# troubling/hummingbird

Measured on AMD Instinct MI355X. Metric: GiB/s device-resident EC encode+reconstruct, 4+2 @ 1 MiB; % HBM roofline, higher is better.
Workload: dtype u8; 1 GPU; 4+2 Encode + Reconstruct{0,1} of 4096 x 1 MiB objects per GPU, device-resident (BASELINE configs[1]+[2]); k=4, m=2, object_bytes=1048576, objects_per_gpu=4096, global_objects=4096, parallelism=object-partition x1

## Files before the change

hummingbird_amd/_native.py:

```python
from __future__ import annotations

import ctypes as C
import os
from pathlib import Path

_PKG = Path(__file__).resolve().parent
LIB_PATH = Path(os.environ.get("HBEC_LIB", _PKG / "libhbec.so"))

HBEC_OK = 0
ERR_INV_SHARD_NUM = -1
ERR_MAX_SHARD_NUM = -2
ERR_TOO_FEW_SHARDS = -3
ERR_SHARD_NO_DATA = -4
ERR_SHARD_SIZE = -5
ERR_SINGULAR = -6
ERR_INVALID_ARG = -7
ERR_DEVICE = -8
ERR_NOMEM = -9
ERR_UNEXPECTED_EOF = -10
ERR_IO = -11
ERR_SCHEME = -12

LOC_BAD = 0x80000000
LOC_SKIPPED = 0x40000000
# ... 73 lines not shown
    ("hbec_plan_stripes", C.c_int, [_P, C.POINTER(Stripe), C.c_uint64, C.POINTER(_P)]),
    ("hbec_plan_objects", C.c_int, [_P, C.POINTER(Object), C.c_uint64, C.POINTER(_P)]),
    ("hbec_plan_free", None, [_P]),
    ("hbec_plan_info", C.c_int,
     [_P, C.POINTER(C.c_uint64), C.POINTER(C.c_int), C.POINTER(C.c_uint64), C.POINTER(C.c_uint64)]),
    ("hbec_encode_plan", C.c_int, [_P, _P, _P]),
    ("hbec_reconstruct_plan", C.c_int, [_P, _P, _U8P, C.c_int, _P]),
    ("hbec_reconstruct_plan_mixed", C.c_int, [_P, _P, _U8P, C.c_uint32, C.POINTER(C.c_uint32), C.c_int, _P]),
    ("hbec_mixed_plan_stats", C.c_int, [C.POINTER(C.c_uint64), C.POINTER(C.c_uint64)]),
    ("hbec_mixed_plan_tile_bytes", C.c_int, []),
    ("hbec_set_mixed_plan_chunk_tiles", C.c_int, [C.c_uint64]),
    ("hbec_verify_plan", C.c_int, [_P, _P, _P, _P]),
    ("hbec_verify_plan_stats", C.c_int, [C.POINTER(C.c_uint64), C.POINTER(C.c_uint64)]),
    ("hbec_verify_plan_tile_bytes", C.c_int, [C.c_int]),
    ("hbec_verify_plan_mixed", C.c_int, [_P, _P, _U8P, C.c_uint32, C.POINTER(C.c_uint32), _P, _P]),
    ("hbec_check_rows", C.c_int,
     [_P, _U8P, C.POINTER(C.c_int), C.POINTER(C.c_int), C.POINTER(C.c_int), _U8P]),
    ("hbec_verify_mixed_plan_stats", C.c_int, [C.POINTER(C.c_uint64), C.POINTER(C.c_uint64)]),
    ("hbec_verify_mixed_plan_tile_bytes", C.c_int, []),
    ("hbec_set_verify_mixed_plan_chunk_tiles", C.c_int, [C.c_uint64]),
    ("hbec_locate_plan_mixed", C.c_int, [_P, _P, _U8P, C.c_uint32, C.POINTER(C.c_uint32), _P, _P, _P]),
    ("hbec_locate_decode", C.c_int, [C.c_int, C.c_int, _U8P, C.c_uint32]),
    ("hbec_locate_plan_stats", C.c_int, [C.POINTER(C.c_uint64), C.POINTER(C.c_uint64)]),
    ("hbec_locate_plan_tile_bytes", C.c_int, []),
    ("hbec_set_locate_plan_chunk_tiles", C.c_int, [C.c_uint64]),
    ("hbec_repair_plan_mixed", C.c_int, [_P, _P, _U8P, C.c_uint32, C.POINTER(C.c_uint32), C.c_int, _P, _P]),
    ("hbec_repair_plan_stats", C.c_int, [C.POINTER(C.c_uint64), C.POINTER(C.c_uint64)]),
    ("hbec_repair_plan_tile_bytes", C.c_int, []),
    ("hbec_set_repair_plan_chunk_tiles", C.c_int, [C.c_uint64]),
    ("hbec_heal_plan_mixed", C.c_int, [_P, _P, _U8P, C.c_uint32, C.POINTER(C.c_uint32), _P, _P, _P]),
    ("hbec_heal_plan_stats", C.c_int, [C.POINTER(C.c_uint64), C.POINTER(C.c_uint64)]),
    ("hbec_heal_plan_tile_bytes", C.c_int, []),
    ("hbec_set_heal_plan_chunk_tiles", C.c_int, [C.c_uint64]),
    ("hbec_verify_host", C.c_int, [_P, C.POINTER(Stripe), C.c_uint64, _U8P]),
    ("hbec_encode_host", C.c_int, [_P, C.POINTER(Stripe), C.c_uint64]),
    ("hbec_host_alloc", C.c_int, [C.c_size_t, C.POINTER(_P)]),
    ("hbec_host_free", None, [_P]),
    ("hbec_host_device_addr", C.c_int, [_P, C.c_uint64, C.POINTER(C.c_uint64)]),
    ("hbec_reconstruct_host", C.c_int, [_P, C.POINTER(Stripe), C.c_uint64, _U8P, C.c_int]),
    ("hbec_encode_host_md5", C.c_int, [_P, C.POINTER(Stripe), C.c_uint64, _U8P]),
    ("hbec_device_count", C.c_int, [C.POINTER(C.c_int)]),
    ("hbec_set_device", C.c_int, [C.c_int]),
    ("hbec_encode_host_devices", C.c_int, [_P, C.POINTER(Stripe), C.c_uint64, C.POINTER(C.c_int), C.c_int]),
    ("hbec_reconstruct_host_devices", C.c_int,
     [_P, C.POINTER(Stripe), C.c_uint64, _U8P, C.c_int, C.POINTER(C.c_int), C.c_int]),
    ("hbec_batcher_new", C.c_int, [_P, C.c_uint64, C.c_uint32, C.POINTER(_P)]),
    ("hbec_batcher_free", None, [_P]),
    ("hbec_batcher_encode", C.c_int, [_P, C.POINTER(Stripe)]),
    ("hbec_batcher_encode_md5", C.c_int, [_P, C.POINTER(Stripe), _U8P]),
    ("hbec_batcher_reconstruct", C.c_int, [_P, C.POINTER(Stripe), _U8P, C.c_int]),
    ("hbec_batcher_stats", C.c_int, [_P, C.POINTER(C.c_uint64), C.POINTER(C.c_uint64)]),
    ("hbec_set_force_stream", C.c_int, [C.c_int]),
    ("hbec_set_odd_chunk_tiles", C.c_int, [C.c_uint64]),
    ("hbec_kernel_info", C.c_int,
     [C.c_int, C.c_int, C.c_uint64, C.POINTER(C.c_int), C.POINTER(C.c_int), C.POINTER(C.c_int)]),
    ("hbec_odd_path_stats", C.c_int, [C.POINTER(C.c_uint64), C.POINTER(C.c_uint64), C.POINTER(C.c_uint64)]),
    ("hbec_verify_route_stats", C.c_int, [C.POINTER(VerifyRoutes)]),
    ("hbec_apply_route_stats", C.c_int, [C.POINTER(ApplyRoutes)]),
    ("hbec_odd_edge_stats", C.c_int, [C.POINTER(C.c_uint64), C.POINTER(C.c_uint64)]),
    ("hbec_odd_record_cache", C.c_int, [C.c_int, C.POINTER(C.c_uint64), C.POINTER(C.c_uint64)]),
    ("hbec_ec_shard_length", C.c_int64, [C.c_int64, C.c_int64]),
    ("hbec_ec_split", C.c_int, [C.c_int, C.c_int, READ_FN, _P, C.c_int, C.c_int64, WRITE_FN, C.POINTER(_P)]),
    ("hbec_ec_reconstruct", C.c_int,
     [C.c_int, C.c_int, READ_FN, C.POINTER(_P), C.c_int, C.c_int64, WRITE_FN, C.POINTER(_P),
      C.POINTER(C.c_int), C.c_int]),
    ("hbec_ec_glue", C.c_int,
     [C.c_int, C.c_int, READ_FN, C.POINTER(_P), C.c_int, C.c_int64, WRITE_FN, C.POINTER(_P), C.c_int]),
    ("hbec_ec_glue_range", C.c_int,
     [C.c_int, C.c_int, READ_FN, C.POINTER(_P), C.c_int, C.c_int64, C.c_int64, C.c_int64, WRITE_FN, C.POINTER(_P),
      C.c_int]),
    ("hbec_ec_copy_range", C.c_int,
     [C.c_int, C.c_int, READ_FN, C.POINTER(_P), C.c_int, C.c_int64, C.c_int64, C.c_int64, WRITE_FN, C.POINTER(_P),
      C.c_int]),
    ("hbec_parse_ec_scheme", C.c_int,
     [C.c_char_p, C.c_char_p, C.c_size_t, C.POINTER(C.c_int64), C.POINTER(C.c_int64), C.POINTER(C.c_int64)]),
    ("hbec_range_chunk_align", None,
     [C.c_int64, C.c_int64, C.c_int64, C.c_int, C.POINTER(C.c_int64), C.POINTER(C.c_int64)]),
]
SYMBOLS = [s[0] for s in _SIG]

_lib = None


class NativeLibraryError(RuntimeError):
    pass


def lib():
    global _lib
    if _lib is None:
        if not LIB_PATH.exists():
            raise NativeLibraryError(
                f"{LIB_PATH} not found: build it with `python -m hummingbird_amd.build` "
                "(there is no CPU fallback)")
        try:
            h = C.CDLL(str(LIB_PATH))
        except OSError as e:
            raise NativeLibraryError(f"cannot load {LIB_PATH}: {e}") from e
        for name, res, args in _SIG:
            if "HBEC_LIB" in os.environ and not hasattr(h, name):
                continue
            fn = getattr(h, name)
            fn.restype = res
            fn.argtypes = args
        _lib = h
    return _lib
# ... 9 lines not shown
```

hummingbird_amd/batch.py:

```python
from __future__ import annotations

import ctypes as C

from . import _native as N
from .reedsolomon import Encoder, check

HBEC_SEED = 0x48424543


def _stream_ptr(stream):
    import torch

    if stream is None:
        stream = torch.cuda.current_stream()
    return C.c_void_p(stream.cuda_stream)


def shard_views(t, n_shards: int, shard_len: int):
    if t.dim() != 2 or t.stride(1) != 1:
        raise ValueError("expected a 2-D row-contiguous tensor")
    if t.shape[1] < n_shards * shard_len:
        raise ValueError("tensor rows shorter than n_shards * shard_len")
    base = t.data_ptr()
    row = t.stride(0) * t.element_size()
# ... 336 lines not shown
    check(N.lib().hbec_mixed_plan_stats(C.byref(a), C.byref(b)))
    return {"kernel_launches": a.value, "per_stripe_calls": b.value}


def mixed_plan_tile_bytes() -> int:
    return int(N.lib().hbec_mixed_plan_tile_bytes())


def set_mixed_plan_chunk_tiles(tiles: int) -> None:
    check(N.lib().hbec_set_mixed_plan_chunk_tiles(int(tiles)))


def verify_mixed_plan_stats():
    a, b = C.c_uint64(), C.c_uint64()
    check(N.lib().hbec_verify_mixed_plan_stats(C.byref(a), C.byref(b)))
    return {"kernel_launches": a.value, "per_stripe_calls": b.value}


def verify_mixed_plan_tile_bytes() -> int:
    return int(N.lib().hbec_verify_mixed_plan_tile_bytes())


def set_verify_mixed_plan_chunk_tiles(tiles: int) -> None:
    check(N.lib().hbec_set_verify_mixed_plan_chunk_tiles(int(tiles)))


KERNEL_KINDS = {0: "unrolled", 1: "pipelined", 2: "streaming", 3: "packed", 4: "records"}


def kernel_info(k: int, r: int, shard_len: int):
    tb, kind, bpc = C.c_int(), C.c_int(), C.c_int()
    check(N.lib().hbec_kernel_info(k, r, int(shard_len), C.byref(tb), C.byref(kind), C.byref(bpc)))
    return {"tile_bytes": tb.value, "kind": KERNEL_KINDS[kind.value], "blocks_per_cu": bpc.value}


def odd_path_stats():
    b, r, s = C.c_uint64(), C.c_uint64(), C.c_uint64()
    check(N.lib().hbec_odd_path_stats(C.byref(b), C.byref(r), C.byref(s)))
    e, f = C.c_uint64(), C.c_uint64()
    check(N.lib().hbec_odd_edge_stats(C.byref(e), C.byref(f)))
    return {"bitplane": b.value, "records": r.value, "strided": s.value, "edges": e.value, "fused": f.value}


def odd_record_cache(clear: bool = False):
    e, h = C.c_uint64(), C.c_uint64()
    check(N.lib().hbec_odd_record_cache(1 if clear else 0, C.byref(e), C.byref(h)))
    return e.value, h.value


def set_odd_chunk_tiles(tiles: int) -> None:
    N.lib().hbec_set_odd_chunk_tiles(int(tiles))


def set_force_stream(on: bool) -> None:
    N.lib().hbec_set_force_stream(1 if on else 0)
```

hummingbird_amd/csrc/hbec.cpp:

```cpp
#include <hip/hip_runtime.h>

#include <algorithm>
#include <atomic>
#include <condition_variable>
#include <cstdio>
#include <cstdlib>
#include <cstring>
#include <deque>
#include <map>
#include <memory>
#include <mutex>
#include <string>
#include <tuple>
#include <vector>

#include "../../include/hbec.h"
#include "gf256.h"
#include "internal.h"
#include "kernels.h"
#include "mixed.h"
#include "vmixed.h"

namespace hbec {

static thread_local std::string t_last_error;

int fail(int code, const std::string& msg) {
    t_last_error = msg;
    return code;
}

int hip_fail(hipError_t e, const char* what) {
    (void)hipGetLastError();
    std::string m = std::string(what) + ": " + hipGetErrorString(e);
    return fail(e == hipErrorOutOfMemory ? HBEC_ERR_NOMEM : HBEC_ERR_DEVICE, m);
}

long long hbec::env_knob(const char* name, long long dflt) {
    const char* e = std::getenv(name);
    return e && *e ? std::atoll(e) : dflt;
}

static std::atomic<int> g_force_stream{0};
static const int g_unaligned_bpc = (int)tune_knob("HBEC_UNALIGNED_BPC", 0);
static const int g_blocks_per_cu_override = (int)tune_knob("HBEC_BLOCKS_PER_CU", 0);
static const int g_grid_cap_env = (int)tune_knob("HBEC_GRID_CAP", 0);
thread_local int t_grid_cap = 0;
void set_thread_grid_cap(int blocks) { t_grid_cap = blocks; }
static int apply_grid_cap(int grid) {
    int cap = g_grid_cap_env;
    if (t_grid_cap > 0) cap = cap > 0 ? std::min(t_grid_cap, cap) : t_grid_cap;
    return cap > 0 ? std::min(grid, cap) : grid;
}
static const uint64_t g_chunk_tiles = [] {
    const long long v = tune_knob("HBEC_CHUNK_TILES", 0);
    return (uint64_t)(v > 0 ? v : (1ll << 20));
}();
static std::atomic<uint64_t> g_odd_chunk_override{0};
static uint64_t odd_chunk_tiles() {
    const uint64_t v = g_odd_chunk_override.load(std::memory_order_relaxed);
    return v ? v : g_chunk_tiles;
}
static const uint64_t g_vec_chunk_tiles = [] {
    const long long v = tune_knob("HBEC_VEC_CHUNK_TILES", tune_knob("HBEC_CHUNK_TILES", 0));
    return (uint64_t)(v > 0 ? v : HBEC_VEC_CHUNK_TILES);
}();

enum class OccKind { Unrolled, Pipelined, ForcedStream, Packed, Unaligned, VerifyPipe, VerifyPacked };

struct DeviceInfo {
    int cus = 0;
    std::map<std::tuple<OccKind, int, int>, int> blocks_per_cu;
};

static std::mutex g_dev_mu;
static std::map<int, DeviceInfo> g_devs;

static int current_device(int* dev) {
    hipError_t e = hipGetDevice(dev);
    if (e != hipSuccess) return hip_fail(e, "hipGetDevice");
    return HBEC_OK;
}

static int device_info(int dev, DeviceInfo** out) {
    DeviceInfo& d = g_devs[dev];
    if (d.cus == 0) {
        hipDeviceProp_t p;
        hipError_t e = hipGetDeviceProperties(&p, dev);
        if (e != hipSuccess) return hip_fail(e, "hipGetDeviceProperties");
        d.cus = p.multiProcessorCount;
    }
    *out = &d;
    return HBEC_OK;
}

int device_cus(int dev, int* cus) {
    std::lock_guard<std::mutex> g(g_dev_mu);
    DeviceInfo* d = nullptr;
    int rc = device_info(dev, &d);
    if (rc) return rc;
    *cus = d->cus;
    return HBEC_OK;
}

static int device_blocks(int dev, OccKind kind, int k, int r, int* cus, int* per_cu) {
    std::lock_guard<std::mutex> g(g_dev_mu);
    DeviceInfo* d = nullptr;
    int rc = device_info(dev, &d);
    if (rc) return rc;
    if (kind == OccKind::Unaligned) k = 0;
    auto it = d->blocks_per_cu.find({kind, k, r});
    if (it == d->blocks_per_cu.end()) {
        int b = 0;
        hipError_t e = hipErrorInvalidValue;
        switch (kind) {
            case OccKind::Unrolled: e = vec_occupancy(k, r, 0, 0, &b); break;
            case OccKind::Pipelined: e = vec_occupancy(k, r, 1, 0, &b); break;
            case OccKind::ForcedStream: e = vec_occupancy(k, r, 0, 1, &b); break;
            case OccKind::Packed: e = packed_occupancy(k, r, &b); break;
// ... 239 lines not shown
                uint64_t n_obj, uint64_t shard_len, hipStream_t stream) {
    if (rows <= 0 || n_obj == 0 || shard_len == 0) return HBEC_OK;
    if (cols <= 0 || !coeffs || !in || !out) return fail(HBEC_ERR_INVALID_ARG, "apply: bad arguments");
    bool vec = vec_len(shard_len);
    for (int c = 0; c < cols && vec; ++c) vec = aligned16(in[c].base) && vec_len(in[c].obj_stride);
    for (int r = 0; r < rows && vec; ++r) vec = aligned16(out[r].base) && vec_len(out[r].obj_stride);
    bool line = vec && shard_len % 128 == 0;
    for (int c = 0; c < cols && line; ++c) line = line_aligned(in[c].base, in[c].obj_stride);
    for (int r = 0; r < rows && line; ++r) line = line_aligned(out[r].base, out[r].obj_stride);
    const bool to_rec = vec && rec_route(cols, rows, shard_len, line, true) &&
                        (rec_route(cols, rows, shard_len, line, false) || bitplane_rows(cols, rows, coeffs, cols, 0, false));
    for (int c = 0; c < cols; ++c)
        if (!in[c].base) return fail(HBEC_ERR_INVALID_ARG, "apply: null input view");
    for (int r = 0; r < rows; ++r)
        if (!out[r].base) return fail(HBEC_ERR_INVALID_ARG, "apply: null output view");
    int dev = 0;
    int rc = current_device(&dev);
    if (rc) return rc;
    const int force_stream = g_force_stream.load();
    if (!vec && cols > kMaxK && cols <= 256 && pos32_shard(shard_len)) {
        count_apply(kArWide);
        return apply_wide(rows, cols, coeffs, in, out, n_obj, shard_len, stream);
    }

    for (int r0 = 0; r0 < rows; r0 += kMaxR) {
        const int R = std::min(kMaxR, rows - r0);
        for (int c0 = 0; c0 < cols; c0 += kMaxK) {
            const int K = std::min(kMaxK, cols - c0);
            PassArgs a = make_pass(in, out, coeffs, cols, r0, R, c0, K, shard_len);
            a.accumulate = c0 > 0 ? 1u : 0u;
            int cus = 0, per_cu = 0;
            if (vec && is_packed_shape(K, R, shard_len, c0 > 0, force_stream)) {
                count_apply(kArPacked);
                rc = device_blocks(dev, OccKind::Packed, K, R, &cus, &per_cu);
                if (rc) return rc;
                if (g_blocks_per_cu_override > 0) per_cu = g_blocks_per_cu_override;
                const uint64_t spo = shard_len / 16;
                const uint64_t te = (uint64_t)packed_tile_elems(K);
                const uint64_t max_obj = packed_objs_per_launch(spo, te, g_chunk_tiles);
                rc = for_object_chunks(a, K, R, n_obj, max_obj, [&](PassArgs& b, uint64_t) {
                    set_packed_tiles(b, spo, te);
                    const int grid = grid_blocks(b.n_tiles, kPipeBlockThreads / 64, (uint64_t)cus * per_cu);
                    return launched(launch_packed(K, R, b, apply_grid_cap(grid), stream), "launch gf_apply_packed");
                });
            } else if (vec && !to_rec) {
                count_apply(kArVec);
                const int pipe = is_pipe_shape(K, R, shard_len, force_stream) && c0 == 0;
                rc = device_blocks(dev, vec_kind(pipe, force_stream), K, R, &cus, &per_cu);
                if (rc) return rc;
                if (g_blocks_per_cu_override > 0) per_cu = g_blocks_per_cu_override;
                const uint64_t tile = (uint64_t)vec_tile_bytes(K, R, shard_len, c0 > 0, force_stream);
                const uint64_t tpo = (shard_len + tile - 1) / tile;
                const uint64_t wpb = (uint64_t)vec_block_threads(K, R, shard_len, c0 > 0, force_stream) / 64;
                const uint64_t max_obj = objs_per_launch(g_vec_chunk_tiles, tpo);
                rc = for_object_chunks(a, K, R, n_obj, max_obj, [&](PassArgs& b, uint64_t) {
                    set_tiles(b, tpo);
                    const int grid = grid_blocks(b.n_tiles, wpb, (uint64_t)cus * per_cu);
                    return launched(launch_vec(K, R, b, apply_grid_cap(grid), stream, force_stream), "launch gf_apply_vec");
                });
            } else if (odd_enabled() && cols <= kOddMaxK && pos32_shard(shard_len)) {
                count_apply(kArOdd);
                rc = odd_launches(a, K, R, 0, c0 > 0, n_obj, shard_len, nullptr, dev, stream);
            } else {
                count_apply(kArUnaligned);
                rc = device_blocks(dev, OccKind::Unaligned, K, R, &cus, &per_cu);
                if (rc) return rc;
                if (g_unaligned_bpc > 0) per_cu = std::min(per_cu, g_unaligned_bpc);
                const uint64_t tpo = unaligned_tiles_per_obj(shard_len);
                const uint64_t max_obj = objs_per_launch(g_chunk_tiles, tpo);
                rc = for_object_chunks(a, K, R, n_obj, max_obj, [&](PassArgs& b, uint64_t) {
                    set_tiles(b, tpo);
                    const int grid = grid_blocks(b.n_tiles, kBlockThreads / 64, (uint64_t)cus * per_cu);
                    return launched(launch_unaligned(K, R, b, apply_grid_cap(grid), stream), "launch gf_apply_unaligned");
                });
            }
            if (rc) return rc;
        }
    }
    return HBEC_OK;
}

struct Staging {
    int dev = 0;
    hipStream_t stream = nullptr;
    uint8_t* dbuf = nullptr;
    size_t dcap = 0;
    uint8_t* hbuf = nullptr;
    uint64_t hbuf_dev = 0;
    size_t hcap = 0;
    std::vector<hipEvent_t> ev;
};

static const bool g_percall_mapped = tune_knob("HBEC_PERCALL_DMA", 0) == 0;

static const int g_percall_pieces = (int)std::max(1LL, std::min(16LL, tune_knob("HBEC_PERCALL_PIECES", 2)));

class PercallGate {
  public:
    explicit PercallGate(int limit) : limit_(limit) {}
    void enter() {
        if (limit_ <= 0) return;
        std::unique_lock<std::mutex> lk(mu_);
        if (running_ < limit_ && waiters_.empty()) {
            ++running_;
            return;
        }
        Waiter w;
        waiters_.push_back(&w);
        w.cv.wait(lk, [&] { return w.granted; });
    }
// ... 995 lines not shown

static void databuf_shards(const hbec_codec* c, uint8_t* databuf, size_t s, std::vector<uint8_t*>& p) {
    p.resize((size_t)(c->k + c->m));
    for (size_t i = 0; i < p.size(); ++i) p[i] = databuf + i * s;
}

int hbec_encode_databuf(hbec_codec* c, uint8_t* databuf, size_t shard_len) {
    return hbec::guarded("hbec_encode_databuf", [&]() -> int {
        if (!c || !databuf) return fail(HBEC_ERR_INVALID_ARG, "null argument");
        if (shard_len == 0) return fail(HBEC_ERR_SHARD_NO_DATA, "no shard data");
        if (coalesce_enabled()) return coalesced_call(c, 0, databuf, shard_len, nullptr, c->k + c->m, 0, kDirect);
        return direct_encode(c, databuf, shard_len);
    });
}

int hbec_reconstruct_databuf(hbec_codec* c, uint8_t* databuf, size_t shard_len, const uint8_t* present,
                             int data_only) {
    return hbec::guarded("hbec_reconstruct_databuf", [&]() -> int {
        if (!c || !databuf || !present) return fail(HBEC_ERR_INVALID_ARG, "null argument");
        std::vector<uint8_t*> p;
        databuf_shards(c, databuf, shard_len, p);
        std::vector<size_t> lens(p.size());
        for (size_t i = 0; i < p.size(); ++i) lens[i] = present[i] ? shard_len : 0;
        return hbec_reconstruct(c, p.data(), lens.data(), (int)p.size(), data_only);
    });
}

int hbec_verify_databuf(hbec_codec* c, const uint8_t* databuf, size_t shard_len, int* ok) {
    return hbec::guarded("hbec_verify_databuf", [&]() -> int {
        if (!c || !databuf || !ok) return fail(HBEC_ERR_INVALID_ARG, "null argument");
        *ok = 0;
        if (shard_len == 0) return fail(HBEC_ERR_SHARD_NO_DATA, "no shard data");
        std::vector<uint8_t*> p;
        databuf_shards(c, const_cast<uint8_t*>(databuf), shard_len, p);
        std::vector<size_t> lens(p.size(), shard_len);
        return hbec_verify(c, p.data(), lens.data(), (int)p.size(), ok);
    });
}

int hbec_coalesce_stats(uint64_t* groups, uint64_t* calls) {
    return hbec::guarded("hbec_coalesce_stats", [&]() -> int {
        coalesce_stats(groups, calls);
        return HBEC_OK;
    });
}

int hbec_set_odd_chunk_tiles(uint64_t tiles) {
    return hbec::guarded("hbec_set_odd_chunk_tiles", [&]() -> int {
        g_odd_chunk_override.store(tiles, std::memory_order_relaxed);
        return HBEC_OK;
    });
}

int hbec_set_force_stream(int on) {
    return hbec::guarded("hbec_set_force_stream", [&]() -> int {
        g_force_stream.store(on ? 1 : 0);
        return HBEC_OK;
    });
}

int hbec_kernel_info(int k, int r, uint64_t shard_len, int* tile_bytes, int* kind, int* blocks_per_cu) {
    return hbec::guarded("hbec_kernel_info", [&]() -> int {
        if (k < 1 || k > kMaxK || r < 1 || r > kMaxR) return fail(HBEC_ERR_INVALID_ARG, "shape out of range");
        const int fs = g_force_stream.load();
        const bool packed = r <= 3 && is_packed_shape(k, r, shard_len, 0, fs);
        const bool rec = !packed && shard_len % 16 == 0 && rec_route(k, r, shard_len, shard_len % 128 == 0, false);
        const int pipe = packed ? 2 : is_pipe_shape(k, r, shard_len, fs);
        if (tile_bytes)
            *tile_bytes = packed ? packed_tile_elems(k) * 16
                                 : (rec ? (int)odd_rec_tile_span(k, 0, -1) : vec_tile_bytes(k, r, shard_len, 0, fs));
        if (kind) *kind = packed ? 3 : (rec ? 4 : (is_streaming_shape(k, r, fs) ? 2 : (pipe ? 1 : 0)));
        if (blocks_per_cu) {
            int dev = 0, cus = 0;
            int rc = current_device(&dev);
            if (rc) return rc;
            rc = device_blocks(dev, packed ? OccKind::Packed : vec_kind(pipe, fs), k, r, &cus, blocks_per_cu);
            if (rc) return rc;
            if (rec) *blocks_per_cu = odd_blocks_per_cu(0, k, r, false, true);
            if (g_blocks_per_cu_override > 0) *blocks_per_cu = g_blocks_per_cu_override;
        }
        return HBEC_OK;
    });
}

}

extern "C" int hbec_odd_record_cache(int clear, uint64_t* entries, uint64_t* hits) {
    return hbec::guarded("hbec_odd_record_cache", [&]() -> int {
        ObjRecCache& C = objrec_cache();
        std::lock_guard<std::mutex> lk(C.mu);
        if (clear) {
            hipError_t e = hipDeviceSynchronize();
            if (e != hipSuccess) return hip_fail(e, "hipDeviceSynchronize (record cache)");
            for (auto& x : C.entries) {
                if (x.ev) (void)hipEventDestroy(x.ev);
                if (x.d) (void)hipFree(x.d);
            }
            C.entries.clear();
            C.seen.clear();
            C.bytes = 0;
            C.hits = 0;
        }
        if (entries) *entries = C.entries.size();
        if (hits) *hits = C.hits;
        return HBEC_OK;
    });
// ... 2 lines not shown
```

hummingbird_amd/csrc/kernels.h:

```cpp
#pragma once
#include <hip/hip_runtime.h>
#include <stdint.h>

#include "tuning.h"

namespace hbec {

long long env_knob(const char* name, long long dflt);
inline long long tune_knob(const char* name, long long dflt) {
#if HBEC_TUNE
    return env_knob(name, dflt);
#else
    (void)name;
    return dflt;
#endif
}

constexpr int kMaxK = 16;
constexpr uint32_t kOddListWords = 4;
constexpr int kMaxR = 4;
constexpr int kBlockThreads = 256;
constexpr int kPipeBlockThreads = HBEC_PIPE_BLOCK;
constexpr int kPipeBlocksPerCu = HBEC_PIPE_BLOCKS_PER_CU;

constexpr int kVecWavesPerSimd = HBEC_WAVES_PER_SIMD;

struct PassArgs {
    const uint8_t* in[kMaxK];
    uint64_t in_stride[kMaxK];
    uint8_t* out[kMaxR];
    uint64_t out_stride[kMaxR];
    uint32_t tab[kMaxR][kMaxK][5];
    uint64_t n_obj;
    uint64_t shard_len;
    uint32_t tiles_per_obj;
    uint32_t n_tiles;
    uint32_t accumulate;
    uint32_t n_elems;
    uint32_t elems_per_obj;
    uint32_t fuse;
    const uint32_t* list;
};

int is_packed_shape(int k, int r, uint64_t shard_len, int accumulate, int force_stream);
int packed_tile_elems(int k);
hipError_t launch_packed(int k, int r, const PassArgs& a, int grid, hipStream_t stream);
hipError_t packed_occupancy(int k, int r, int* blocks_per_cu);

int vec_tile_bytes(int k, int r, uint64_t shard_len, int accumulate, int force_stream);
int is_streaming_shape(int k, int r, int force_stream);
int is_pipe_shape(int k, int r, uint64_t shard_len, int force_stream);
int vec_block_threads(int k, int r, uint64_t shard_len, int accumulate, int force_stream);
__host__ __device__ constexpr int pipe_u(int k) { return k <= 4 ? (4 / k) : (k <= 8 ? HBEC_PIPE_U_BIG : 1); }

__host__ __device__ constexpr int stripes_u(int k) { return k <= 4 ? pipe_u(k) : 1; }
__host__ __device__ constexpr int verify_u(int k) { return k <= 4 ? 4 : 1; }

hipError_t launch_vec(int k, int r, const PassArgs& a, int grid, hipStream_t stream, int force_stream);
uint32_t unaligned_tiles_per_obj(uint64_t shard_len);
hipError_t launch_unaligned(int k, int r, const PassArgs& a, int grid, hipStream_t stream);
hipError_t unaligned_occupancy(int r, int* blocks_per_cu);
struct URec {
    uint64_t a;
    uint64_t b;
    uint64_t shard_len;
    uint64_t p0;
};
struct UPlanArgs {
    const URec* recs;
    uint32_t n_recs;
    uint32_t accumulate;
    uint32_t in_idx[kMaxK];
    uint32_t out_idx[kMaxR];
    uint32_t in_sel, out_sel;
    uint32_t tab[kMaxR][kMaxK][5];
    uint32_t mirror;
    uint32_t carry;
};
uint32_t unaligned_tile_bytes();
hipError_t launch_verify_unaligned(int k, int r, const PassArgs& a, uint32_t* flags, int grid, hipStream_t stream);
hipError_t launch_unaligned_plan(int k, int r, const UPlanArgs& a, int grid, hipStream_t stream);
constexpr int kOddMaxK = 12;
constexpr uint64_t kPos32MaxShard = (1ull << 31) - (1ull << 16);
__host__ __device__ constexpr bool pos32_shard(uint64_t shard_len) { return shard_len <= kPos32MaxShard; }
bool odd_enabled();
int odd_blocks_per_cu(int mode, int k, int r, bool mirror = false, bool records = false, int xs = -1);
bool odd_supported(int k, int r);
uint64_t urec_tile();
uint64_t urec_tile_for(int k, bool mirror);
uint64_t urec_span(uint64_t shard_len);
uint32_t odd_tile_bytes(int k);
uint32_t odd_plan_tile_bytes();
uint32_t odd_tiles_per_obj(int k, int mode, uint64_t shard_len, bool records, int xs = -1);
uint64_t odd_frame_tiles(uint64_t shard_len, uint64_t tile);
int odd_bp_schedule(int k, int r, int mode, const uint32_t (*tab)[kMaxK][5], bool plan);
uint32_t odd_rec_tile_span(int k, int mode, int xs);
uint32_t odd_waves_per_block(int xs);
uint64_t odd_min_main();
bool odd_uses_records(int k, int r);
uint32_t odd_rec_words(int k, int r, int mode);
hipError_t launch_odd_objrec(int k, int r, int mode, const PassArgs& a, uint32_t* recs, hipStream_t stream);
hipError_t launch_odd_planrec(int k, int r, int mode, const UPlanArgs& p, const URec* orecs, uint32_t n,
                              uint32_t* recs, hipStream_t stream);
hipError_t launch_odd(int k, int r, int mode, const PassArgs& a, uint32_t* flags, const uint32_t* recs, int grid,
                      hipStream_t stream, int xs = -1);
bool odd_edge_fuse(int k, int r, int mode, bool records, int xs, bool list, uint64_t max_s);
// ... 80 lines not shown
```

hummingbird_amd/csrc/kernels.hip:

```cpp
#include <hip/hip_runtime.h>
#include <stdint.h>

#include <cstdlib>
#include <cstring>

#include "gf_device.h"
#include "kernels.h"

namespace hbec {

template <int K, int R, int U>
__device__ __forceinline__ void process_tile(const PassArgs& a, const Tables<K, R>& tb, uint64_t obj,
                                             uint64_t off0, bool full, bool accumulate) {
    u32x4 x[U][K];
    const uint64_t last = a.shard_len - 16u;
#pragma unroll
    for (int u = 0; u < U; ++u) {
        uint64_t off = off0 + (uint64_t)u * 1024u;
        if (!full) off = off < last ? off : last;
#pragma unroll
        for (int j = 0; j < K; ++j) x[u][j] = ld16(a.in[j] + obj * a.in_stride[j] + off);
    }
    u32x4 old[U][R];
    if (accumulate) {
// ... 139 lines not shown
#pragma unroll
    for (int r = 0; r < R; ++r) b.out[r] = reinterpret_cast<uint64_t>(a.out[r]) + obj * a.out_stride[r] + off;
    const uint64_t left = a.shard_len - off;
    b.valid = (uint32_t)(left < TILE ? left : TILE);
    b.live = b.valid;
}

template <int K, int R, int U>
__device__ __forceinline__ void pipe2_load(u32x4 (&x)[U][K], const PipeTile<K, R>& b, uint32_t lane) {
    const uint64_t last = (uint64_t)b.valid - 16u;
#pragma unroll
    for (int q = 0; q < U * K; ++q) {
        const int u = HBEC_PIPE_IMAJ ? q % U : q / K, j = HBEC_PIPE_IMAJ ? q / U : q % K;
        uint64_t off = (uint64_t)lane * 16u + (uint64_t)u * 1024u;
        off = off < last ? off : last;
        x[u][j] = HBEC_PIPE_TEMP ? ld16_addr_t(b.in[j] + off) : ld16_addr(b.in[j] + off);
    }
}

template <int K, int R, int U, bool FULL>
__device__ __forceinline__ void pipe2_store_(const u32x4 (&x)[U][K], const PassArgs& a, const Tables<K, R>& tb,
                                             const PipeTile<K, R>& b, uint32_t lane) {
#pragma unroll
    for (int u = 0; u < U; ++u) {
        const uint64_t off = (uint64_t)lane * 16u + (uint64_t)u * 1024u;
        u32x4 acc[R];
#pragma unroll
        for (int r = 0; r < R; ++r) acc[r] = u32x4{0, 0, 0, 0};
        gf_dot<K, R>(acc, x[u], a.tab, tb);
        if (FULL || off < b.live) {
#pragma unroll
            for (int r = 0; r < R; ++r) st16_addr(b.out[r] + off, acc[r]);
        }
    }
}

template <int K, int R, int U>
__device__ __forceinline__ void pipe_tile_at(PipeTile<K, R>& b, const PassArgs& a, uint32_t t, uint32_t n,
                                             uint32_t tpo) {
    pipe_tile_coords<K, R, U>(b, a, t < n ? t : n - 1u, tpo);
    if (t >= n) b.live = 0;
}

template <int K, int R, int U>
__device__ __forceinline__ void pipe2_finish(const u32x4 (&x)[U][K], const PassArgs& a, const Tables<K, R>& tb,
                                             const PipeTile<K, R>& cur, uint32_t lane) {
    if (cur.live >= (uint32_t)U * 1024u)
        pipe2_store_<K, R, U, true>(x, a, tb, cur, lane);
    else
        pipe2_store_<K, R, U, false>(x, a, tb, cur, lane);
}


template <int K, int R>
__global__ __launch_bounds__(kPipeBlockThreads, 1) void gf_apply_vec_pipe2(PassArgs a) {
    constexpr int U = pipe_u(K);
    constexpr uint32_t WPB = kPipeBlockThreads / 64;
    const uint32_t lane = threadIdx.x & 63u;
    const uint32_t nw = gridDim.x * WPB;
    const uint32_t wave0 = __builtin_amdgcn_readfirstlane(xcd_block() * WPB);
    const uint32_t dw = __builtin_amdgcn_readfirstlane(threadIdx.x >> 6);
    const uint32_t wave = wave0 + dw;
    const uint32_t tpo = a.tiles_per_obj;
    const uint32_t n = a.n_tiles;
    if (wave0 >= n) return;
    const Tables<K, R> tb = load_tables<K, R>(a.tab);
    PipeTile<K, R> cur, nxt;
    pipe_tile_at<K, R, U>(cur, a, wave, n, tpo);
    u32x4 x[U][K];
    pipe2_load<K, R, U>(x, cur, lane);
    pipe_tile_at<K, R, U>(nxt, a, wave + nw, n, tpo);
    for (uint32_t b0 = wave0 + nw; b0 < n; b0 += nw) {
        u32x4 y[U][K];
        pipe2_load<K, R, U>(y, nxt, lane);
        if (K <= 4) __builtin_amdgcn_s_sleep(HBEC_PIPE2_SLEEP);
        __builtin_amdgcn_s_barrier();
        PipeTile<K, R> after;
        pipe_tile_at<K, R, U>(after, a, b0 + dw + nw, n, tpo);
        pipe2_finish<K, R, U>(x, a, tb, cur, lane);
#pragma unroll
        for (int u = 0; u < U; ++u)
#pragma unroll
            for (int j = 0; j < K; ++j) x[u][j] = y[u][j];
        cur = nxt;
        nxt = after;
    }
    pipe2_finish<K, R, U>(x, a, tb, cur, lane);
}

template <int K, int U>
__device__ __forceinline__ void packed_load(u32x4 (&x)[U][K], const PassArgs& a, const PackedCoord<U>& c) {
#pragma unroll
    for (int u = 0; u < U; ++u)
#pragma unroll
        for (int j = 0; j < K; ++j) x[u][j] = ld16(a.in[j] + (uint64_t)c.obj[u] * a.in_stride[j] + c.off[u]);
}

template <int K, int R, int U, bool FULL>
__device__ __forceinline__ void packed_store_(const u32x4 (&x)[U][K], const PassArgs& a, const Tables<K, R>& tb,
                                              const PackedCoord<U>& c, uint32_t t, uint32_t lane, uint32_t live) {
#pragma unroll
    for (int u = 0; u < U; ++u) {
        u32x4 acc[R];
#pragma unroll
        for (int r = 0; r < R; ++r) acc[r] = u32x4{0, 0, 0, 0};
        gf_dot<K, R>(acc, x[u], a.tab, tb);
        if (FULL || (t * (uint32_t)U + (uint32_t)u) * 64u + lane < live) {
#pragma unroll
            for (int r = 0; r < R; ++r) st16(a.out[r] + (uint64_t)c.obj[u] * a.out_stride[r] + c.off[u], acc[r]);
        }
    }
}

template <int K, int R, int U>
__device__ __forceinline__ void packed_finish(const u32x4 (&x)[U][K], const PassArgs& a, const Tables<K, R>& tb,
                                              const PackedCoord<U>& c, uint32_t t, uint32_t n, uint32_t lane) {
    const uint32_t live = t < n ? a.n_elems : 0u;
    if (t < n && (t + 1u) * (uint32_t)U * 64u <= a.n_elems)
        packed_store_<K, R, U, true>(x, a, tb, c, t, lane, live);
    else
        packed_store_<K, R, U, false>(x, a, tb, c, t, lane, live);
}


__host__ __device__ constexpr int packed_u(int k) {
    return k > 4 ? HBEC_PACKED_U_BIG : pipe_u(k);
}

template <int K, int R>
__global__ __launch_bounds__(kPipeBlockThreads, 1) void gf_apply_packed(PassArgs a) {
    constexpr int U = packed_u(K);
// ... 572 lines not shown
```

hummingbird_amd/csrc/tuning.h:

```cpp
#pragma once

#ifndef HBEC_TUNE
#define HBEC_TUNE 0
#endif

#ifndef HBEC_PIPE_BLOCK
#define HBEC_PIPE_BLOCK 256
#endif
#ifndef HBEC_PIPE_BLOCKS_PER_CU
#define HBEC_PIPE_BLOCKS_PER_CU 1
#endif
#ifndef HBEC_PIPE_U_BIG
#define HBEC_PIPE_U_BIG 3
#endif
#ifndef HBEC_PIPE_SLEEP
#define HBEC_PIPE_SLEEP 6
#endif
#ifndef HBEC_PIPE2_SLEEP
#define HBEC_PIPE2_SLEEP 8
#endif
#ifndef HBEC_PIPE_IMAJ
#define HBEC_PIPE_IMAJ 0
#endif
#ifndef HBEC_PIPE_TEMP
#define HBEC_PIPE_TEMP 0
#endif
#ifndef HBEC_VEC_CHUNK_TILES
#define HBEC_VEC_CHUNK_TILES 262144
#endif
#ifndef HBEC_PIPE_V2_MAXK
#define HBEC_PIPE_V2_MAXK 4
#endif

#ifndef HBEC_WAVES_PER_SIMD
#define HBEC_WAVES_PER_SIMD 4
#endif
#ifndef HBEC_TILE_SMALL
#define HBEC_TILE_SMALL 4
#endif
#ifndef HBEC_TILE_MID
#define HBEC_TILE_MID 1
#endif
#ifndef HBEC_TILE_BIG
#define HBEC_TILE_BIG 1
#endif

#ifndef HBEC_ALLVGPR_MIN
#define HBEC_ALLVGPR_MIN 16
#endif

#ifndef HBEC_PACKED_U_BIG
#define HBEC_PACKED_U_BIG 1
#endif
#ifndef HBEC_PACKED_MAX_BIG
#define HBEC_PACKED_MAX_BIG 32784
#endif
#ifndef HBEC_PACKED_BLOCKS_SMALL
#define HBEC_PACKED_BLOCKS_SMALL 2
#endif
#ifndef HBEC_PACKED_BLOCKS_BIG
#define HBEC_PACKED_BLOCKS_BIG 1
#endif
#ifndef HBEC_VERIFY_PACKED_U_SMALL
#define HBEC_VERIFY_PACKED_U_SMALL 2
#endif
#ifndef HBEC_VERIFY_PACKED_U_BIG
#define HBEC_VERIFY_PACKED_U_BIG 1
#endif
#ifndef HBEC_VERIFY_PACKED_BLOCKS_SMALL
#define HBEC_VERIFY_PACKED_BLOCKS_SMALL 2
#endif
#ifndef HBEC_VERIFY_PACKED_BLOCKS_BIG
// ... 89 lines not shown
```

include/hbec.h:

```cpp
#ifndef HBEC_H
#define HBEC_H

#include <stddef.h>
#include <stdint.h>

#ifdef __cplusplus
extern "C" {
#endif


#define HBEC_VERSION 2

enum {
    HBEC_OK = 0,
    HBEC_ERR_INV_SHARD_NUM = -1,
    HBEC_ERR_MAX_SHARD_NUM = -2,
    HBEC_ERR_TOO_FEW_SHARDS = -3,
    HBEC_ERR_SHARD_NO_DATA = -4,
    HBEC_ERR_SHARD_SIZE = -5,
    HBEC_ERR_SINGULAR = -6,
    HBEC_ERR_INVALID_ARG = -7,
    HBEC_ERR_DEVICE = -8,
    HBEC_ERR_NOMEM = -9,
    HBEC_ERR_UNEXPECTED_EOF = -10,
// ... 111 lines not shown
#define HBEC_LOC_BAD 0x80000000u
#define HBEC_LOC_SKIPPED 0x40000000u
#define HBEC_LOC_NOTHING 0x20000000u
int hbec_locate_plan_mixed(hbec_codec* codec, const hbec_plan* plan, const uint8_t* patterns, uint32_t n_patterns,
                           const uint32_t* pattern_of, const uint32_t* d_flags ,
                           uint32_t* d_where, void* hip_stream);
#define HBEC_LOC_CLEAN (-1)
#define HBEC_LOC_AMBIGUOUS (-2)
#define HBEC_LOC_MULTIPLE (-3)
#define HBEC_LOC_UNCHECKED (-4)
int hbec_locate_decode(int k, int m, const uint8_t* present, uint32_t where);
int hbec_locate_plan_stats(uint64_t* kernel_launches, uint64_t* skipped_entries);
int hbec_locate_plan_tile_bytes(void);
int hbec_set_locate_plan_chunk_tiles(uint64_t tiles);
int hbec_repair_plan_mixed(hbec_codec* codec, const hbec_plan* plan, const uint8_t* patterns, uint32_t n_patterns,
                           const uint32_t* pattern_of, int data_only, uint32_t* d_flags, void* hip_stream);
int hbec_repair_plan_stats(uint64_t* kernel_launches, uint64_t* per_stripe_calls);
int hbec_repair_plan_tile_bytes(void);
int hbec_set_repair_plan_chunk_tiles(uint64_t tiles);
#define HBEC_HEAL_DONE 4u
#define HBEC_HEAL_UNNAMED 8u
int hbec_heal_plan_mixed(hbec_codec* codec, const hbec_plan* plan, const uint8_t* patterns, uint32_t n_patterns,
                         const uint32_t* pattern_of, const uint32_t* d_where, uint32_t* d_flags, void* hip_stream);
int hbec_heal_plan_stats(uint64_t* kernel_launches, uint64_t* skipped_entries);
int hbec_heal_plan_tile_bytes(void);
int hbec_set_heal_plan_chunk_tiles(uint64_t tiles);

int hbec_encode_host(hbec_codec* codec, const hbec_stripe* stripes, uint64_t n_stripes);
int hbec_host_alloc(size_t bytes, void** out);
void hbec_host_free(void* p);
int hbec_host_device_addr(const void* p, uint64_t len, uint64_t* dev);
int hbec_reconstruct_host(hbec_codec* codec, const hbec_stripe* stripes, uint64_t n_stripes, const uint8_t* present,
                          int data_only);
int hbec_verify_host(hbec_codec* codec, const hbec_stripe* stripes, uint64_t n_stripes, uint8_t* flags);
int hbec_device_count(int* n);
int hbec_set_device(int device);
int hbec_encode_host_devices(hbec_codec* codec, const hbec_stripe* stripes, uint64_t n_stripes, const int* devices,
                             int n_devices);
int hbec_reconstruct_host_devices(hbec_codec* codec, const hbec_stripe* stripes, uint64_t n_stripes,
                                  const uint8_t* present, int data_only, const int* devices, int n_devices);
int hbec_encode_host_md5(hbec_codec* codec, const hbec_stripe* stripes, uint64_t n_stripes, uint8_t* digests);
int hbec_host_md5_stats(uint64_t* zero_copy_calls, uint64_t* ring_calls);

typedef struct hbec_batcher hbec_batcher;
int hbec_batcher_new(hbec_codec* codec, uint64_t max_batch_bytes, uint32_t max_wait_us, hbec_batcher** out);
void hbec_batcher_free(hbec_batcher* batcher);
int hbec_batcher_encode(hbec_batcher* batcher, const hbec_stripe* stripe);
int hbec_batcher_encode_md5(hbec_batcher* batcher, const hbec_stripe* stripe, uint8_t* digests);
int hbec_batcher_reconstruct(hbec_batcher* batcher, const hbec_stripe* stripe, const uint8_t* present, int data_only);
int hbec_batcher_stats(hbec_batcher* batcher, uint64_t* batches, uint64_t* stripes);

int hbec_set_force_stream(int on);
int hbec_set_odd_chunk_tiles(uint64_t tiles);
int hbec_kernel_info(int k, int r, uint64_t shard_len, int* tile_bytes, int* kind, int* blocks_per_cu);
int hbec_odd_path_stats(uint64_t* bitplane, uint64_t* records, uint64_t* strided);
typedef struct hbec_verify_routes {
    uint64_t packed, pipe, records, odd, wide, unaligned, scratch;
} hbec_verify_routes;
int hbec_verify_route_stats(hbec_verify_routes* out);
typedef struct hbec_apply_routes {
    uint64_t packed, vec, odd, unaligned, wide;
} hbec_apply_routes;
int hbec_apply_route_stats(hbec_apply_routes* out);

int hbec_odd_edge_stats(uint64_t* edge_launches, uint64_t* fused_launches);

int hbec_odd_record_cache(int clear, uint64_t* entries, uint64_t* hits);

typedef int64_t (*hbec_read_fn)(void* ctx, uint8_t* buf, size_t n);
typedef int (*hbec_write_fn)(void* ctx, const uint8_t* buf, size_t n);

int64_t hbec_ec_shard_length(int64_t length, int64_t data_shards);

int hbec_ec_split(int data_shards, int parity_shards, hbec_read_fn read, void* fp, int chunk_size,
                  int64_t content_length, hbec_write_fn write, void* const* writers);

int hbec_ec_reconstruct(int data_shards, int parity_shards, hbec_read_fn read, void* const* bodies, int chunk_size,
                        int64_t content_length, hbec_write_fn write, void* const* dsts, const int* dst_chunk_num,
                        int n_dsts);

int hbec_ec_glue(int data_shards, int parity_shards, hbec_read_fn read, void* const* bodies, int chunk_size,
                 int64_t content_length, hbec_write_fn write, void* const* dsts, int n_dsts);

int hbec_ec_glue_range(int data_shards, int parity_shards, hbec_read_fn read, void* const* bodies, int chunk_size,
                       int64_t content_length, int64_t start, int64_t end, hbec_write_fn write, void* const* dsts,
                       int n_dsts);

int hbec_ec_copy_range(int data_shards, int parity_shards, hbec_read_fn read, void* const* bodies, int chunk_size,
                       int64_t content_length, int64_t start, int64_t end, hbec_write_fn write, void* const* dsts,
                       int n_dsts);

int hbec_parse_ec_scheme(const char* scheme, char* algo, size_t algo_cap, int64_t* data_shards,
                         int64_t* parity_shards, int64_t* chunk_size);

void hbec_range_chunk_align(int64_t start, int64_t end, int64_t chunk_size, int data_shards, int64_t* out_start,
                            int64_t* out_end);

#ifdef __cplusplus
}
#endif
#endif
```

Measured before the change: 5530 GiB/s.

## Batch pipe2 stores two tiles deep with contiguous per-wave tile runs for 4+2

For the k=4, r=2 pipelined vector apply kernel, results from T consecutive tiles are accumulated in registers and written back in one burst. A run-based tile mapping gives each wave contiguous groups of T tiles. The intent is to cut interleaving between loads and stores on HBM and to improve DRAM locality for writes, at the cost of extra VGPR pressure from holding T tiles of accumulators. The change also adds runtime setters for the vec chunk size and grid cap, plus query functions, for tuning.

New measurement: 5953 GiB/s (median of 6 runs). 7.6% higher.

```diff
diff --git a/hummingbird_amd/_native.py b/hummingbird_amd/_native.py
--- a/hummingbird_amd/_native.py
+++ b/hummingbird_amd/_native.py
@@ -149,6 +149,10 @@
     ("hbec_batcher_stats", C.c_int, [_P, C.POINTER(C.c_uint64), C.POINTER(C.c_uint64)]),
     ("hbec_set_force_stream", C.c_int, [C.c_int]),
     ("hbec_set_odd_chunk_tiles", C.c_int, [C.c_uint64]),
+    ("hbec_set_vec_chunk_tiles", C.c_int, [C.c_uint64]),
+    ("hbec_set_vec_grid_cap", C.c_int, [C.c_int]),
+    ("hbec_vec_launch_config", C.c_int, [C.POINTER(C.c_uint64), C.POINTER(C.c_int)]),
+    ("hbec_pipe2_store_depth", C.c_int, [C.c_int, C.c_int, C.POINTER(C.c_int), C.POINTER(C.c_int)]),
     ("hbec_kernel_info", C.c_int,
      [C.c_int, C.c_int, C.c_uint64, C.POINTER(C.c_int), C.POINTER(C.c_int), C.POINTER(C.c_int)]),
     ("hbec_odd_path_stats", C.c_int, [C.POINTER(C.c_uint64), C.POINTER(C.c_uint64), C.POINTER(C.c_uint64)]),
diff --git a/hummingbird_amd/batch.py b/hummingbird_amd/batch.py
--- a/hummingbird_amd/batch.py
+++ b/hummingbird_amd/batch.py
@@ -412,5 +412,25 @@
     N.lib().hbec_set_odd_chunk_tiles(int(tiles))
 
 
+def set_vec_chunk_tiles(tiles: int) -> None:
+    check(N.lib().hbec_set_vec_chunk_tiles(int(tiles)))
+
+
+def set_vec_grid_cap(blocks: int) -> None:
+    check(N.lib().hbec_set_vec_grid_cap(int(blocks)))
+
+
+def vec_launch_config() -> tuple[int, int]:
+    t, g = C.c_uint64(), C.c_int()
+    check(N.lib().hbec_vec_launch_config(C.byref(t), C.byref(g)))
+    return t.value, g.value
+
+
+def pipe2_store_depth(k: int, r: int) -> tuple[int, bool]:
+    d, run = C.c_int(), C.c_int()
+    check(N.lib().hbec_pipe2_store_depth(k, r, C.byref(d), C.byref(run)))
+    return d.value, bool(run.value)
+
+
 def set_force_stream(on: bool) -> None:
     N.lib().hbec_set_force_stream(1 if on else 0)
diff --git a/hummingbird_amd/csrc/hbec.cpp b/hummingbird_amd/csrc/hbec.cpp
--- a/hummingbird_amd/csrc/hbec.cpp
+++ b/hummingbird_amd/csrc/hbec.cpp
@@ -65,6 +65,16 @@
     const long long v = tune_knob("HBEC_VEC_CHUNK_TILES", tune_knob("HBEC_CHUNK_TILES", 0));
     return (uint64_t)(v > 0 ? v : HBEC_VEC_CHUNK_TILES);
 }();
+static std::atomic<uint64_t> g_vec_chunk_override{0};
+static std::atomic<int> g_vec_grid_cap{0};
+static uint64_t vec_chunk_tiles() {
+    const uint64_t v = g_vec_chunk_override.load(std::memory_order_relaxed);
+    return v ? v : g_vec_chunk_tiles;
+}
+static int vec_grid_cap(int grid) {
+    const int cap = g_vec_grid_cap.load(std::memory_order_relaxed);
+    return cap > 0 ? std::min(grid, cap) : grid;
+}
 
 enum class OccKind { Unrolled, Pipelined, ForcedStream, Packed, Unaligned, VerifyPipe, VerifyPacked };
 
@@ -410,10 +420,10 @@
                 const uint64_t tile = (uint64_t)vec_tile_bytes(K, R, shard_len, c0 > 0, force_stream);
                 const uint64_t tpo = (shard_len + tile - 1) / tile;
                 const uint64_t wpb = (uint64_t)vec_block_threads(K, R, shard_len, c0 > 0, force_stream) / 64;
-                const uint64_t max_obj = objs_per_launch(g_vec_chunk_tiles, tpo);
+                const uint64_t max_obj = objs_per_launch(vec_chunk_tiles(), tpo);
                 rc = for_object_chunks(a, K, R, n_obj, max_obj, [&](PassArgs& b, uint64_t) {
                     set_tiles(b, tpo);
-                    const int grid = grid_blocks(b.n_tiles, wpb, (uint64_t)cus * per_cu);
+                    const int grid = vec_grid_cap(grid_blocks(b.n_tiles, wpb, (uint64_t)cus * per_cu));
                     return launched(launch_vec(K, R, b, apply_grid_cap(grid), stream, force_stream), "launch gf_apply_vec");
                 });
             } else if (odd_enabled() && cols <= kOddMaxK && pos32_shard(shard_len)) {
@@ -1515,6 +1525,40 @@
     });
 }
 
+int hbec_set_vec_chunk_tiles(uint64_t tiles) {
+    return hbec::guarded("hbec_set_vec_chunk_tiles", [&]() -> int {
+        if (tiles > (1ull << 31)) return fail(HBEC_ERR_INVALID_ARG, "vec chunk tiles: at most 2^31");
+        g_vec_chunk_override.store(tiles, std::memory_order_relaxed);
+        return HBEC_OK;
+    });
+}
+
+int hbec_set_vec_grid_cap(int blocks) {
+    return hbec::guarded("hbec_set_vec_grid_cap", [&]() -> int {
+        if (blocks < 0) return fail(HBEC_ERR_INVALID_ARG, "vec grid cap: negative");
+        g_vec_grid_cap.store(blocks, std::memory_order_relaxed);
+        return HBEC_OK;
+    });
+}
+
+int hbec_vec_launch_config(uint64_t* chunk_tiles, int* grid_cap) {
+    return hbec::guarded("hbec_vec_launch_config", [&]() -> int {
+        if (chunk_tiles) *chunk_tiles = vec_chunk_tiles();
+        if (grid_cap) *grid_cap = g_vec_grid_cap.load(std::memory_order_relaxed);
+        return HBEC_OK;
+    });
+}
+
+int hbec_pipe2_store_depth(int k, int r, int* depth, int* run) {
+    return hbec::guarded("hbec_pipe2_store_depth", [&]() -> int {
+        if (k < 1 || k > kMaxK || r < 1 || r > kMaxR) return fail(HBEC_ERR_INVALID_ARG, "shape out of range");
+        const int t = k <= HBEC_PIPE_V2_MAXK && r <= 3 ? pipe2_store_depth(k, r) : 1;
+        if (depth) *depth = t;
+        if (run) *run = t > 1 && HBEC_PIPE2_RUN != 0 ? 1 : 0;
+        return HBEC_OK;
+    });
+}
+
 int hbec_set_force_stream(int on) {
     return hbec::guarded("hbec_set_force_stream", [&]() -> int {
         g_force_stream.store(on ? 1 : 0);
diff --git a/hummingbird_amd/csrc/kernels.h b/hummingbird_amd/csrc/kernels.h
--- a/hummingbird_amd/csrc/kernels.h
+++ b/hummingbird_amd/csrc/kernels.h
@@ -52,6 +52,13 @@
 int is_pipe_shape(int k, int r, uint64_t shard_len, int force_stream);
 int vec_block_threads(int k, int r, uint64_t shard_len, int accumulate, int force_stream);
 __host__ __device__ constexpr int pipe_u(int k) { return k <= 4 ? (4 / k) : (k <= 8 ? HBEC_PIPE_U_BIG : 1); }
+
+__host__ __device__ constexpr int pipe2_store_depth(int k, int r) {
+    return (k == 4 && r == 2 && HBEC_PIPE2_STORE_DEPTH > 1)
+               ? (HBEC_PIPE2_STORE_DEPTH * pipe_u(k) * r * 4 <= 128 ? HBEC_PIPE2_STORE_DEPTH
+                                                                    : 128 / (pipe_u(k) * r * 4))
+               : 1;
+}
 
 __host__ __device__ constexpr int stripes_u(int k) { return k <= 4 ? pipe_u(k) : 1; }
 __host__ __device__ constexpr int verify_u(int k) { return k <= 4 ? 4 : 1; }
diff --git a/hummingbird_amd/csrc/kernels.hip b/hummingbird_amd/csrc/kernels.hip
--- a/hummingbird_amd/csrc/kernels.hip
+++ b/hummingbird_amd/csrc/kernels.hip
@@ -215,31 +215,107 @@
 }
 
 
+template <int K, int R, int U, int T, bool FULL>
+__device__ __forceinline__ void pipe2_burst(const u32x4 (&acc)[T][U][R], const uint64_t (&dst)[T][R],
+                                            const int32_t (&room)[T]) {
+#pragma unroll
+    for (int s = 0; s < T; ++s)
+#pragma unroll
+        for (int u = 0; u < U; ++u) {
+            if (FULL || u * 1024 < room[s]) {
+#pragma unroll
+                for (int r = 0; r < R; ++r) st16_addr(dst[s][r] + (uint64_t)u * 1024u, acc[s][u][r]);
+            }
+        }
+}
+
 template <int K, int R>
 __global__ __launch_bounds__(kPipeBlockThreads, 1) void gf_apply_vec_pipe2(PassArgs a) {
     constexpr int U = pipe_u(K);
+    constexpr int T = pipe2_store_depth(K, R);
+    constexpr bool RUN = T > 1 && HBEC_PIPE2_RUN != 0;
     constexpr uint32_t WPB = kPipeBlockThreads / 64;
     const uint32_t lane = threadIdx.x & 63u;
     const uint32_t nw = gridDim.x * WPB;
     const uint32_t wave0 = __builtin_amdgcn_readfirstlane(xcd_block() * WPB);
     const uint32_t dw = __builtin_amdgcn_readfirstlane(threadIdx.x >> 6);
-    const uint32_t wave = wave0 + dw;
     const uint32_t tpo = a.tiles_per_obj;
     const uint32_t n = a.n_tiles;
-    if (wave0 >= n) return;
+    const auto tile_of = [&](uint32_t i) -> uint32_t {
+        if (RUN) {
+            const uint32_t q = i / (uint32_t)T;
+            return (q * nw + wave0) * (uint32_t)T + (i - q * (uint32_t)T) * WPB + dw;
+        }
+        return wave0 + dw + i * nw;
+    };
+    uint32_t rows;
+    if (RUN) {
+        const uint32_t span = nw * (uint32_t)T, q = n / span, rem = n - q * span, lo = wave0 * (uint32_t)T;
+        const uint32_t part = rem > lo ? (rem - lo + WPB - 1u) / WPB : 0u;
+        rows = q * (uint32_t)T + (part < (uint32_t)T ? part : (uint32_t)T);
+    } else {
+        rows = wave0 < n ? (n - wave0 + nw - 1u) / nw : 0u;
+    }
+    if (rows == 0) return;
+    const uint32_t steps = rows - 1u;
     const Tables<K, R> tb = load_tables<K, R>(a.tab);
     PipeTile<K, R> cur, nxt;
-    pipe_tile_at<K, R, U>(cur, a, wave, n, tpo);
+    pipe_tile_at<K, R, U>(cur, a, tile_of(0), n, tpo);
     u32x4 x[U][K];
     pipe2_load<K, R, U>(x, cur, lane);
-    pipe_tile_at<K, R, U>(nxt, a, wave + nw, n, tpo);
-    for (uint32_t b0 = wave0 + nw; b0 < n; b0 += nw) {
+    pipe_tile_at<K, R, U>(nxt, a, tile_of(1), n, tpo);
+    uint32_t i = 0;
+    if constexpr (T > 1) {
+        for (uint32_t g = steps / (uint32_t)T; g > 0; --g) {
+            u32x4 acc[T][U][R];
+            uint64_t dst[T][R];
+            int32_t room[T];
+            bool full = true;
+#pragma unroll
+            for (int s = 0; s < T; ++s) {
+                u32x4 y[U][K];
+                pipe2_load<K, R, U>(y, nxt, lane);
+                if (K <= 4) __builtin_amdgcn_s_sleep(HBEC_PIPE2_SLEEP);
+                __builtin_amdgcn_s_barrier();
+                __builtin_amdgcn_sched_barrier(0);
+                PipeTile<K, R> after;
+                pipe_tile_at<K, R, U>(after, a, tile_of(i + 2u), n, tpo);
+#pragma unroll
+                for (int u = 0; u < U; ++u) {
+#pragma unroll
+                    for (int r = 0; r < R; ++r) acc[s][u][r] = u32x4{0, 0, 0, 0};
+                    gf_dot<K, R>(acc[s][u], x[u], a.tab, tb);
+                }
+#pragma unroll
+                for (int r = 0; r < R; ++r) dst[s][r] = cur.out[r] + (uint64_t)lane * 16u;
+                room[s] = (int32_t)cur.live - (int32_t)(lane * 16u);
+                full = full && cur.live >= (uint32_t)U * 1024u;
+#pragma unroll
+                for (int u = 0; u < U; ++u)
+#pragma unroll
+                    for (int r = 0; r < R; ++r) asm volatile("" : "+v"(acc[s][u][r]));
+                __builtin_amdgcn_sched_barrier(0);
+#pragma unroll
+                for (int u = 0; u < U; ++u)
+#pragma unroll
+                    for (int j = 0; j < K; ++j) x[u][j] = y[u][j];
+                cur = nxt;
+                nxt = after;
+                ++i;
+            }
+            if (full)
+                pipe2_burst<K, R, U, T, true>(acc, dst, room);
+            else
+                pipe2_burst<K, R, U, T, false>(acc, dst, room);
+        }
+    }
+    for (; i < steps; ++i) {
         u32x4 y[U][K];
         pipe2_load<K, R, U>(y, nxt, lane);
         if (K <= 4) __builtin_amdgcn_s_sleep(HBEC_PIPE2_SLEEP);
         __builtin_amdgcn_s_barrier();
         PipeTile<K, R> after;
-        pipe_tile_at<K, R, U>(after, a, b0 + dw + nw, n, tpo);
+        pipe_tile_at<K, R, U>(after, a, tile_of(i + 2u), n, tpo);
         pipe2_finish<K, R, U>(x, a, tb, cur, lane);
 #pragma unroll
         for (int u = 0; u < U; ++u)
diff --git a/hummingbird_amd/csrc/tuning.h b/hummingbird_amd/csrc/tuning.h
--- a/hummingbird_amd/csrc/tuning.h
+++ b/hummingbird_amd/csrc/tuning.h
@@ -18,6 +18,12 @@
 #endif
 #ifndef HBEC_PIPE2_SLEEP
 #define HBEC_PIPE2_SLEEP 8
+#endif
+#ifndef HBEC_PIPE2_STORE_DEPTH
+#define HBEC_PIPE2_STORE_DEPTH 2
+#endif
+#ifndef HBEC_PIPE2_RUN
+#define HBEC_PIPE2_RUN 1
 #endif
 #ifndef HBEC_PIPE_IMAJ
 #define HBEC_PIPE_IMAJ 0
diff --git a/include/hbec.h b/include/hbec.h
--- a/include/hbec.h
+++ b/include/hbec.h
@@ -187,6 +187,10 @@
 
 int hbec_set_force_stream(int on);
 int hbec_set_odd_chunk_tiles(uint64_t tiles);
+int hbec_set_vec_chunk_tiles(uint64_t tiles);
+int hbec_set_vec_grid_cap(int blocks);
+int hbec_vec_launch_config(uint64_t* chunk_tiles, int* grid_cap);
+int hbec_pipe2_store_depth(int k, int r, int* depth, int* run);
 int hbec_kernel_info(int k, int r, uint64_t shard_len, int* tile_bytes, int* kind, int* blocks_per_cu);
 int hbec_odd_path_stats(uint64_t* bitplane, uint64_t* records, uint64_t* strided);
 typedef struct hbec_verify_routes {
```
